# Gibbs-liu/PuzzleNet

Measured on NVIDIA B200. Metric: pairs/sec PuzzleNet fwd B=64 N=1024, higher is better.
Workload: dtype f16x3 (fp16 hi/lo operand planes, 3 tcgen05 MMAs per product, fp32 accumulate)

## Files before the change

puzzlenet_b200/csrc/encoder.cu:

```cuda
#include <stdlib.h>

#include <functional>

#include <cuda_fp16.h>

#include "pz_common.cuh"
#include "se3_math.cuh"

namespace pz {

constexpr int NPTS = 1024;
constexpr int S1 = 512, S2 = 256, KNN = 32;
constexpr int D0 = 64, C1A = 128, C1B = 128, C2A = 256, C2B = 256, LATT = 256, CATT = 256;

struct StemW {
  const float *w1, *b1, *w2, *b2;
  const float *g1, *be1, *m1, *v1, *g2, *be2, *m2, *v2;
};

__global__ void __launch_bounds__(128) stem_kernel(const float* __restrict__ xyz, StemW wa, StemW wb,
                                                   int clouds_per_set, float* __restrict__ out,
                                                   __nv_bfloat16* __restrict__ out_b, __half* __restrict__ out_hi,
                                                   __half* __restrict__ out_lo) {
  __shared__ __align__(16) float w2s[64 * 64];
  __shared__ float w1s[64 * 3], b1s[64], b2s[64];
  const size_t p = (size_t)blockIdx.x * 128 + threadIdx.x;
  const int cloud = (int)(p / NPTS);
  const int n = (int)(p - (size_t)cloud * NPTS);
  const StemW& w = (cloud / clouds_per_set) == 0 ? wa : wb;
  for (int i = threadIdx.x; i < 64 * 64; i += 128) w2s[i] = w.w2[i];
  for (int i = threadIdx.x; i < 64 * 3; i += 128) w1s[i] = w.w1[i];
  if (threadIdx.x < 64) {
    b1s[threadIdx.x] = w.b1[threadIdx.x];
    b2s[threadIdx.x] = w.b2[threadIdx.x];
  }
  __syncthreads();
  const float a1 = w.g1[n] * (1.0f / sqrtf(w.v1[n] + 1e-5f));
  const float c1 = w.be1[n] - w.m1[n] * a1;
  const float a2 = w.g2[n] * (1.0f / sqrtf(w.v2[n] + 1e-5f));
  const float c2 = w.be2[n] - w.m2[n] * a2;
  const float x = xyz[p * 3], y = xyz[p * 3 + 1], z = xyz[p * 3 + 2];
  float h[64];
#pragma unroll
  for (int k = 0; k < 64; ++k) {
    float v = b1s[k];
    v = fmaf(w1s[k * 3 + 0], x, v);
    v = fmaf(w1s[k * 3 + 1], y, v);
    v = fmaf(w1s[k * 3 + 2], z, v);
    h[k] = fmaxf(fmaf(v, a1, c1), 0.f);
  }
  float* o = out + p * 64;
// ... 1206 lines not shown
      prof_mark("attn_out_proj", st);
    }
  }
  {
    float* fg = o.f_global ? o.f_global : s.fglob;
    TcGemm g;
    g.X = cat_b; g.ldx = 1280; g.W[0] = wpa + WP_WOUT; g.W[1] = wpb + WP_WOUT; g.ldw = 1280;
    g.bias[0] = wa.out_b; g.bias[1] = wb.out_b; g.rows_per_wset = B * LATT; g.M = rows; g.Nout = 1024; g.K = 1280;
    if (o.out) {
      g.Yf = o.out; g.ldyf = 1024;
      PZ_TRY(launch_tc_gemm(g, st));
      prof_mark("tail_linear", st);
      rowblock_max_kernel<<<dim3(4, C), 256, 0, st>>>(o.out, 1024, LATT, 1024, C, C, 0, fg, 1024);
      PZ_LAUNCH_CHECK();
      prof_mark("tail_point_max", st);
    } else {
      g.epi = 2; g.Yf = fg; g.ldyf = 1024;
      PZ_TRY(launch_tc_gemm(g, st));
      prof_mark("tail_linear_maxpool", st);
    }
    if (fglob_pair)
      PZ_CUDA(cudaMemcpy2DAsync(fglob_pair, (size_t)E * 1024 * sizeof(float), fg, 1024 * sizeof(float),
                                1024 * sizeof(float), B, cudaMemcpyDeviceToDevice, st));
    if (fglob_pair && E == 2)
      PZ_CUDA(cudaMemcpy2DAsync(fglob_pair + 1024, (size_t)E * 1024 * sizeof(float), fg + (size_t)B * 1024,
                                1024 * sizeof(float), 1024 * sizeof(float), B, cudaMemcpyDeviceToDevice, st));
  }
  return 0;
}


static int encoder_forward_split(const PzEncoderWeights* w, int E, int B, const float* xyz, const int64_t* start1,
                                 const int64_t* start2, const PzEncoderOutputs& o, EncoderScratch& s, float* fglob_pair,
                                 const float** xfeat_out, const AfterStem* after_stem, bool reuse_pack, cudaStream_t st) {
  const int C = E * B;
  const PzEncoderWeights& wa = w[0];
  const PzEncoderWeights& wb = w[E - 1];
  float* xfeat = o.x_feature ? o.x_feature : s.xfeat;
  float* nx2 = o.x2 ? o.x2 : s.nx2;
  if (xfeat_out) *xfeat_out = xfeat;
  typedef __nv_bfloat16 h16;
  h16* xfeat_h[2] = {s.P1, s.P1 + (size_t)C * NPTS * D0};
  float* P1 = s.F1;
  float* P2 = s.F2;
  float* Q1 = s.v;
  float* Q2 = s.r;
  h16* f1f_h[2] = {s.f1f_b, s.Q1};
  h16* cat_h[2] = {s.att_cat_b, reinterpret_cast<h16*>(s.att_cat)};
  h16* qk_h[2] = {s.qk_b, reinterpret_cast<h16*>(s.q)};
  h16* vT_h[2] = {s.vT_b, s.P2};
  h16* r_h[2] = {s.r_b, s.Q2};

  if (!reuse_pack) {
    PackJobs jobs;
    int n = 0;
    auto add = [&](const float* src, int ldi, int rows, int cols, void* dst, int ldo, int mode) {
      if (n < MAX_PACK_JOBS) jobs.j[n] = PackJob{src, dst, ldi, rows, cols, ldo, mode};
      ++n;
    };
    for (int e = 0; e < E; ++e) {
      const PzEncoderWeights& we = w[e];
      for (int pl = 0; pl < 2; ++pl) {
        h16* wp = s.wpack + (size_t)(e * 2 + pl) * WS_TOTAL;
        const int mode = 4 + pl;
        add(we.mlp3_w + 3, 3 + D0, C1A, D0, wp + WS_W3F, D0, mode);
        add(we.mlp4_w, C1A, C1B, C1A, wp + WS_W4, C1A, mode);
        add(we.mlp5_w + 3, 3 + C1B, C2A, C1B, wp + WS_W5F, C1B, mode);
// ... 24 lines not shown
                          {s.wpack + (size_t)(E - 1) * 2 * WS_TOTAL, s.wpack + ((size_t)(E - 1) * 2 + 1) * WS_TOTAL}};
  auto set_w = [&](TcGemm& g, size_t off) {
    g.W[0] = wp_[0][0] + off; g.Wlo[0] = wp_[0][1] + off; g.W[1] = wp_[1][0] + off; g.Wlo[1] = wp_[1][1] + off;
  };

  PZ_CUDA(cudaMemsetAsync(s.tailp, 0, (size_t)3 * C * sizeof(int), st));

  SideStream* ss = nullptr;
  PZ_TRY(side_stream(&ss, st));
  static const bool env_serial = getenv("PZ_SIDE_STREAM") == nullptr || getenv("PZ_NO_SIDE_STREAM") != nullptr;
  const bool serial = env_serial || prof_serial();
  cudaStream_t sg = serial ? st : ss->stream;
  const int gl = serial ? 0 : 1;
  if (!serial) {
    PZ_CUDA(cudaEventRecord(ss->fork, st));
    PZ_CUDA(cudaStreamWaitEvent(sg, ss->fork, 0));
  }
  prof_mark("_side_begin", sg, gl);
  PZ_TRY(launch_fps(xyz, C, NPTS, start1, S1, o.fps1, nullptr, s.nx1, sg));
  prof_mark("fps1", sg, gl);
  PZ_TRY(launch_knn(s.nx1, xyz, C, S1, NPTS, KNN, o.knn1, s.knn1r, nullptr, sg));
  prof_mark("knn1", sg, gl);
  PZ_TRY(launch_centre_proj_f32(s.nx1, wa.mlp3_w, wb.mlp3_w, 3 + D0, B * S1, C * S1, C1A, Q1, sg));
  if (!serial) PZ_CUDA(cudaEventRecord(ss->join_a, sg));
  PZ_TRY(launch_fps(s.nx1, C, S1, start2, S2, o.fps2, nullptr, nx2, sg));
  prof_mark("fps2", sg, gl);
  PZ_TRY(launch_knn(nx2, s.nx1, C, S2, S1, KNN, o.knn2, s.knn2r, nullptr, sg));
  prof_mark("knn2", sg, gl);
  PZ_TRY(launch_centre_proj_f32(nx2, wa.mlp5_w, wb.mlp5_w, 3 + C1B, B * S2, C * S2, C2A, Q2, sg));
  if (!serial) PZ_CUDA(cudaEventRecord(ss->join_b, sg));

  static const bool stem_ffma = getenv("PZ_STEM_FFMA") && getenv("PZ_STEM_FFMA")[0] == '1';
  const int reps = head_reps();
  if (stem_ffma || (C * NPTS) % (128 * reps) != 0) {
    stem_kernel<<<C * NPTS / 128, 128, 0, st>>>(xyz, stem_of(wa), stem_of(wb), B, xfeat, nullptr, nullptr, nullptr);
    PZ_LAUNCH_CHECK();
    PZ_TRY(launch_split_planes(xfeat, D0, (size_t)C * NPTS, D0, xfeat_h[0], xfeat_h[1], D0, st));
  } else {
    PZ_CUDA(cudaFuncSetAttribute(stem_tc_kernel<true>, cudaFuncAttributeMaxDynamicSharedMemorySize, (int)STEM_TC_SMEM));
    PZ_CUDA(launch_pdl(stem_tc_kernel<true>, dim3(C * NPTS / (128 * reps)), dim3(128), STEM_TC_SMEM, st, xyz, stem_of(wa), stem_of(wb),
                       (const __nv_bfloat16*)nullptr, (const __nv_bfloat16*)nullptr, B, reps, xfeat,
                       reinterpret_cast<__nv_bfloat16*>(xfeat_h[0]), reinterpret_cast<__half*>(xfeat_h[1])));
    PZ_LAUNCH_CHECK();
  }
  prof_mark("stem", st);
  {
    TcGemm g;
    g.X = xfeat_h[0]; g.Xlo = xfeat_h[1]; g.ldx = D0; set_w(g, WS_W3F); g.ldw = D0;
    g.bias[0] = wa.mlp3_b; g.bias[1] = wb.mlp3_b; g.rows_per_wset = B * NPTS; g.M = C * NPTS; g.Nout = C1A; g.K = D0;
    g.Yf = P1; g.ldyf = C1A; g.xyz = xyz; g.W1x[0] = wa.mlp3_w; g.W1x[1] = wb.mlp3_w; g.ldw1x = 3 + D0;
    PZ_TRY(launch_split_rowgemm(g, st));
    prof_mark("sg1_layer1", st);
  }
  if (after_stem) PZ_TRY((*after_stem)(xfeat, nullptr));
  if (!serial) PZ_CUDA(cudaStreamWaitEvent(st, ss->join_a, 0));
  prof_mark("_wait_geometry1", st);
  {
    TcGemm g;
    g.Xf = P1; g.ldx = C1A; g.Qf = Q1; g.rows = s.knn1r; set_w(g, WS_W4); g.ldw = C1A;
    g.bias[0] = wa.mlp4_b; g.bias[1] = wb.mlp4_b; g.rows_per_wset = B * S1 * KNN; g.M = C * S1 * KNN; g.Nout = C1B;
    g.K = C1A; g.epi = 1; g.relu = 1; g.Yf = o.f1f; g.ldyf = C1B; g.Yb = f1f_h[0]; g.Yblo = f1f_h[1]; g.ldyb = C1B;
    PZ_TRY(launch_split_gather(g, st));
    prof_mark("sg1_gather_layer2_maxpool", st);
  }
  {
    TcGemm g;
    g.X = f1f_h[0]; g.Xlo = f1f_h[1]; g.ldx = C1B; set_w(g, WS_W5F); g.ldw = C1B;
    g.bias[0] = wa.mlp5_b; g.bias[1] = wb.mlp5_b; g.rows_per_wset = B * S1; g.M = C * S1; g.Nout = C2A; g.K = C1B;
    g.Yf = P2; g.ldyf = C2A; g.xyz = s.nx1; g.W1x[0] = wa.mlp5_w; g.W1x[1] = wb.mlp5_w; g.ldw1x = 3 + C1B;
    PZ_TRY(launch_split_rowgemm(g, st));
    prof_mark("sg2_layer1", st);
  }
  if (!serial) PZ_CUDA(cudaStreamWaitEvent(st, ss->join_b, 0));
  prof_mark("_wait_geometry2", st);
  float* cat_f = o.att_cat;
  {
    TcGemm g;
    g.Xf = P2; g.ldx = C2A; g.Qf = Q2; g.rows = s.knn2r; set_w(g, WS_W6); g.ldw = C2A;
    g.bias[0] = wa.mlp6_b; g.bias[1] = wb.mlp6_b; g.rows_per_wset = B * S2 * KNN; g.M = C * S2 * KNN; g.Nout = C2B;
    g.K = C2A; g.epi = 1; g.relu = 1; g.Yb = cat_h[0] + 4 * CATT; g.Yblo = cat_h[1] + 4 * CATT; g.ldyb = 1280;
    if (cat_f) { g.Yf = cat_f + 4 * CATT; g.ldyf = 1280; }
    else if (o.f2f) { g.Yf = o.f2f; g.ldyf = CATT; }
    PZ_TRY(launch_split_gather(g, st));
    prof_mark("sg2_gather_layer2_maxpool", st);
  }
  if (o.f2f && cat_f)
    PZ_CUDA(cudaMemcpy2DAsync(o.f2f, CATT * sizeof(float), cat_f + 4 * CATT, 1280 * sizeof(float), CATT * sizeof(float),
// ... 51 lines not shown
    g.X = r_h[0]; g.Xlo = r_h[1]; g.ldx = CATT; set_w(g, wl + 384 * CATT); g.ldw = CATT;
    g.bias[0] = wa.o_b[l]; g.bias[1] = wb.o_b[l]; g.rows_per_wset = B * LATT; g.M = rows; g.Nout = CATT; g.K = CATT;
    g.relu = 1; g.Rb = cat_h[0] + xoff; g.Rblo = cat_h[1] + xoff; g.ldrb = 1280;
    g.Yb = cat_h[0] + (size_t)l * CATT; g.Yblo = cat_h[1] + (size_t)l * CATT; g.ldyb = 1280;
    if (cat_f) { g.Yf = cat_f + (size_t)l * CATT; g.ldyf = 1280; }
    PZ_TRY(launch_split_rowgemm(g, st));
    prof_mark("attn_out_proj", st);
  }
  {
    float* fg = o.f_global ? o.f_global : s.fglob;
    TcGemm g;
    g.X = cat_h[0]; g.Xlo = cat_h[1]; g.ldx = 1280; set_w(g, WS_WOUT); g.ldw = 1280;
    g.bias[0] = wa.out_b; g.bias[1] = wb.out_b; g.rows_per_wset = B * LATT; g.M = rows; g.Nout = 1024; g.K = 1280;
    if (o.out) { g.Yf = o.out; g.ldyf = 1024; }
    g.Ymax = s.tailp; g.ldmax = 1024;
    PZ_TRY(launch_split_rowgemm(g, st));
    prof_mark("tail_linear_maxpool", st);
    PZ_CUDA(launch_pdl(rowblock_max_kernel, dim3(4, C), dim3(256), 0, st, (const float*)s.tailp, 1024, LATT / 128, 1024, C, C, 0, fg, 1024));
    PZ_LAUNCH_CHECK();
    prof_mark("tail_point_max", st);
    if (fglob_pair)
      PZ_CUDA(cudaMemcpy2DAsync(fglob_pair, (size_t)E * 1024 * sizeof(float), fg, 1024 * sizeof(float),
                                1024 * sizeof(float), B, cudaMemcpyDeviceToDevice, st));
    if (fglob_pair && E == 2)
      PZ_CUDA(cudaMemcpy2DAsync(fglob_pair + 1024, (size_t)E * 1024 * sizeof(float), fg + (size_t)B * 1024,
                                1024 * sizeof(float), 1024 * sizeof(float), B, cudaMemcpyDeviceToDevice, st));
  }
  return 0;
}

static int encoder_forward_impl(const PzEncoderWeights* w, int E, int B, const float* xyz, const int64_t* start1,
                                const int64_t* start2, int precision, const PzEncoderOutputs& o, void* ws,
                                size_t ws_bytes, float* fglob_pair, const float** xfeat_out, const AfterStem* after_stem,
                                bool reuse_pack, cudaStream_t st) {
  PZ_REQUIRE(E == 1 || E == 2, PZ_ERR_ARG, "encoder: E must be 1 or 2 (got %d)", E);
  PZ_REQUIRE(B >= 1, PZ_ERR_ARG, "encoder: B must be >= 1");
  PZ_REQUIRE(precision == PZ_PREC_FP32 || precision == PZ_PREC_BF16 || precision == PZ_PREC_SPLIT, PZ_ERR_ARG,
             "encoder: unknown precision %d", precision);
  for (int e = 0; e < E; ++e)
    PZ_REQUIRE(encoder_weights_ok(w[e]), PZ_ERR_ARG, "encoder: weight set %d has a null pointer", e);
  const int C = E * B;
  Arena arena(ws, ws_bytes);
  EncoderScratch s;
  encoder_scratch_layout(C, arena, s);
  PZ_REQUIRE(ws && arena.ok(), PZ_ERR_WORKSPACE, "encoder: workspace %zu B < required %zu B", ws_bytes, arena.used);
  if (precision == PZ_PREC_BF16)
    return encoder_forward_bf16(w, E, B, xyz, start1, start2, o, s, fglob_pair, xfeat_out, after_stem, reuse_pack, st);
  if (precision == PZ_PREC_SPLIT)
    return encoder_forward_split(w, E, B, xyz, start1, start2, o, s, fglob_pair, xfeat_out, after_stem, reuse_pack, st);
  const PzEncoderWeights& wa = w[0];
  const PzEncoderWeights& wb = w[E - 1];
  float* xfeat = o.x_feature ? o.x_feature : s.xfeat;
  float* f1f = o.f1f ? o.f1f : s.f1f;
  float* att_cat = o.att_cat ? o.att_cat : s.att_cat;
  float* nx2 = o.x2 ? o.x2 : s.nx2;
  if (xfeat_out) *xfeat_out = xfeat;

  stem_kernel<<<C * NPTS / 128, 128, 0, st>>>(xyz, stem_of(wa), stem_of(wb), B, xfeat, nullptr, nullptr, nullptr);
  PZ_LAUNCH_CHECK();
  prof_mark("stem", st);
  if (after_stem) PZ_TRY((*after_stem)(xfeat, nullptr));

  PZ_TRY(launch_fps(xyz, C, NPTS, start1, S1, o.fps1, nullptr, s.nx1, st));
  prof_mark("fps1", st);
  PZ_TRY(launch_knn(s.nx1, xyz, C, S1, NPTS, KNN, o.knn1, s.knn1r, nullptr, st));
  prof_mark("knn1", st);
  {
    GemmF32 g;
    g.A = xfeat; g.lda = D0; g.W[0] = wa.mlp3_w + 3; g.W[1] = wb.mlp3_w + 3; g.ldw = 3 + D0;
    g.rows_per_wset = B * NPTS; g.Y = s.F1; g.ldy = C1A; g.M = C * NPTS; g.N = C1A; g.K = D0;
    PZ_TRY(launch_gemm_f32(g, st));
    prof_mark("sg1_layer1", st);
  }
  {
    GemmF32 g;
    g.A = s.F1; g.lda = C1A; g.rows = s.knn1r; g.xyz = xyz; g.centers = s.nx1;
    g.W1[0] = wa.mlp3_w; g.W1[1] = wb.mlp3_w; g.b1[0] = wa.mlp3_b; g.b1[1] = wb.mlp3_b; g.ldw1 = 3 + D0;
    g.W[0] = wa.mlp4_w; g.W[1] = wb.mlp4_w; g.bias[0] = wa.mlp4_b; g.bias[1] = wb.mlp4_b; g.ldw = C1A;
    g.rows_per_wset = B * S1 * KNN; g.Y = f1f; g.ldy = C1B; g.M = C * S1 * KNN; g.N = C1B; g.K = C1A;
    g.relu = 1; g.group = 32;
    PZ_TRY(launch_gemm_f32(g, st));
    prof_mark("sg1_gather_layer2_maxpool", st);
// ... 64 lines not shown
      prof_mark("tail_linear_maxpool", st);
      rowblock_max_kernel<<<dim3(4, C), 256, 0, st>>>(s.tailp, 1024, LATT / 128, 1024, C, C, 0, fg, 1024);
    }
    PZ_LAUNCH_CHECK();
    prof_mark("tail_point_max", st);
    if (fglob_pair)
      PZ_CUDA(cudaMemcpy2DAsync(fglob_pair, (size_t)E * 1024 * sizeof(float), fg, 1024 * sizeof(float),
                                1024 * sizeof(float), B, cudaMemcpyDeviceToDevice, st));
    if (fglob_pair && E == 2)
      PZ_CUDA(cudaMemcpy2DAsync(fglob_pair + 1024, (size_t)E * 1024 * sizeof(float), fg + (size_t)B * 1024,
                                1024 * sizeof(float), 1024 * sizeof(float), B, cudaMemcpyDeviceToDevice, st));
  }
  return 0;
}

}

using namespace pz;

extern "C" size_t pz_encoder_workspace_bytes(int E, int B) {
  if (E < 1 || B < 1) return 0;
  Arena a(nullptr, 0);
  EncoderScratch s;
  return align_up(encoder_scratch_layout(E * B, a, s), 256);
}

extern "C" int pz_encoder_forward(const PzEncoderWeights* weights_host, int E, int B, const float* xyz,
                                  const int64_t* start1, const int64_t* start2, int precision,
                                  const PzEncoderOutputs* outputs_host, void* workspace, size_t workspace_bytes,
                                  pz_stream_t stream) {
  PZ_REQUIRE(weights_host && xyz && start1 && start2 && outputs_host, PZ_ERR_ARG, "pz_encoder_forward: null pointer");
  prof_begin(as_stream(stream));
  return encoder_forward_impl(weights_host, E, B, xyz, start1, start2, precision, *outputs_host, workspace,
                              workspace_bytes, nullptr, nullptr, nullptr, false, as_stream(stream));
}

namespace {
struct PredictScratch {
  float *xyz, *fpair, *h0, *h1, *partial, *local, *gmax, *gbias, *tilemax;
  __nv_bfloat16 *ha, *himg, *himg_split;
  int64_t *st1, *st2;
  void* enc;
  size_t enc_bytes, partial_floats;
};
size_t predict_layout(int B, Arena& a, PredictScratch& s) {
  s.xyz = a.take<float>((size_t)2 * B * NPTS * 3);
  s.st1 = a.take<int64_t>((size_t)2 * B);
  s.st2 = a.take<int64_t>((size_t)2 * B);
  s.fpair = a.take<float>((size_t)B * 2048);
  s.h0 = a.take<float>((size_t)B * 1024);
  s.h1 = a.take<float>((size_t)B * 1024);
  s.partial_floats = (size_t)16 * B * 1024;
  s.partial = a.take<float>(s.partial_floats);
  s.local = a.take<float>((size_t)2 * B * NPTS * 64);
  s.gmax = a.take<float>((size_t)B * 64);
  s.gbias = a.take<float>((size_t)2 * B * 64);
  s.tilemax = a.take<float>((size_t)2 * B * 8 * 128);
  s.ha = a.take<__nv_bfloat16>((size_t)2 * B * NPTS * 64);
  s.himg = a.take<__nv_bfloat16>(2 * HEAD_IMG_SET);
  s.himg_split = a.take<__nv_bfloat16>(2 * HEAD_SPLIT_IMG_SET);
  s.enc_bytes = pz_encoder_workspace_bytes(2, B);
  s.enc = a.take<char>(s.enc_bytes);
  return a.used;
}
}

namespace pz {
// ... 98 lines not shown
          jobs.j[n++] = PackJob{pre.w2, wp + 128 * HD_WS, 64, 64, 64, HD_WS, 1};
          jobs.j[n++] = PackJob{seg.w0 + 64, wp + 192 * HD_WS, 128, 64, 64, HD_WS, 1};
          jobs.j[n++] = PackJob{seg.w1, wp + 256 * HD_WS, 64, 32, 64, HD_WS, 1};
          jobs.j[n++] = PackJob{seg.w1, wp + 288 * HD_WS, 64, 32, 64, HD_WS, 3};
        }
        jobs.n = n;
        pack_weights_kernel<<<dim3(16, n), 256, 0, st>>>(jobs);
        PZ_LAUNCH_CHECK();
      }
      head_pre_tc_kernel<<<P / (128 * head_reps()), 128, 0, st>>>(xfeat_b, pre_f, pre_r, s.himg, B, head_reps(), s.ha, s.tilemax);
      PZ_LAUNCH_CHECK();
      head_seg_tc_kernel<<<P / (128 * head_reps()), 128, 0, st>>>(s.ha, seg_f, seg_r, s.himg, B, head_reps(), s.tilemax, de_fpcb,
                                                                  de_mrpcb);
      PZ_LAUNCH_CHECK();
      prof_mark("boundary_heads", st);
      return 0;
    }
    const size_t hl_smem = (3 * 4160 + 64 * 128) * sizeof(float);
    const size_t hs_smem = (64 * 64 + 32 * 64 + 64 + 32 + 64 + 4 + 64 * 128) * sizeof(float);
    PZ_CUDA(cudaFuncSetAttribute(head_seg_kernel, cudaFuncAttributeMaxDynamicSharedMemorySize, (int)hs_smem));
    PZ_CUDA(cudaFuncSetAttribute(head_local_kernel, cudaFuncAttributeMaxDynamicSharedMemorySize, (int)hl_smem));
    head_local_kernel<<<P / 128, 128, hl_smem, st>>>(xfeat, pre_f, pre_r, B, s.local);
    PZ_LAUNCH_CHECK();
    rowblock_max_kernel<<<dim3(1, B), 256, 0, st>>>(s.local + (size_t)B * NPTS * 64, 64, NPTS, 64, B, B, 0, s.gmax, 64);
    PZ_LAUNCH_CHECK();
    seg_bias_kernel<<<dim3(B, 2), 64, 0, st>>>(s.gmax, h.seg_fpc_w[0], h.seg_fpc_b[0], h.seg_rpc_w[0], h.seg_rpc_b[0], B, s.gbias);
    PZ_LAUNCH_CHECK();
    head_seg_kernel<<<P / 128, 128, hs_smem, st>>>(s.local, seg_f, seg_r, s.gbias, B, de_fpcb, de_mrpcb);
    PZ_LAUNCH_CHECK();
    prof_mark("boundary_heads", st);
    return 0;
  };

  const float* xfeat = nullptr;
  PZ_TRY(encoder_forward_impl(enc_host, 2, B, s.xyz, s.st1, s.st2, precision, eo, s.enc, s.enc_bytes, s.fpair,
                              &xfeat, &heads_fn, reuse_pack, st));
  if (need) {
    const size_t ab = (size_t)B * LATT * LATT * sizeof(float), xb = (size_t)B * S2 * 3 * sizeof(float);
    PZ_CUDA(cudaMemcpyAsync(attention_fpc, attn_all, ab, cudaMemcpyDeviceToDevice, st));
    PZ_CUDA(cudaMemcpyAsync(attention_mrpc, attn_all + (size_t)B * LATT * LATT, ab, cudaMemcpyDeviceToDevice, st));
    PZ_CUDA(cudaMemcpyAsync(x2_fpc, x2_all, xb, cudaMemcpyDeviceToDevice, st));
    PZ_CUDA(cudaMemcpyAsync(x2_mrpc, x2_all + (size_t)B * S2 * 3, xb, cudaMemcpyDeviceToDevice, st));
  }
  PZ_TRY(skinny_linear(s.fpair, 2048, h.tf_w[0], h.tf_b[0], B, 1024, 2048, 1, s.h0, 1024, s.partial, s.partial_floats, st));
  PZ_TRY(skinny_linear(s.h0, 1024, h.tf_w[1], h.tf_b[1], B, 512, 1024, 1, s.h1, 512, s.partial, s.partial_floats, st));
  PZ_TRY(skinny_linear(s.h1, 512, h.tf_w[2], h.tf_b[2], B, 512, 512, 1, s.h0, 512, s.partial, s.partial_floats, st));
  PZ_TRY(skinny_linear(s.h0, 512, h.tf_w[3], h.tf_b[3], B, 256, 512, 1, s.h1, 256, s.partial, s.partial_floats, st));
  PZ_TRY(skinny_linear(s.h1, 256, h.tf_w[4], h.tf_b[4], B, 6, 256, 0, out6, 6, s.partial, s.partial_floats, st));
  prof_mark("pose_mlp", st);
  return 0;
}

extern "C" int pz_se3_exp(const float* twist, int B, float* g, pz_stream_t stream) {
  PZ_REQUIRE(twist && g, PZ_ERR_ARG, "pz_se3_exp: null pointer");
  PZ_REQUIRE(B >= 0, PZ_ERR_ARG, "pz_se3_exp: B < 0");
  if (B == 0) return 0;
  se3_exp_kernel<<<(B + 127) / 128, 128, 0, as_stream(stream)>>>(twist, B, g);
  PZ_LAUNCH_CHECK();
  return 0;
}

extern "C" int pz_scaled_dot_attention(const float* q, const float* k, const float* v, int B, int L, int Dk, int Dv,
                                       float* values, float* attention_or_null, pz_stream_t stream) {
  PZ_REQUIRE(q && k && v && values, PZ_ERR_ARG, "pz_scaled_dot_attention: null pointer");
  PZ_REQUIRE(B >= 0, PZ_ERR_ARG, "pz_scaled_dot_attention: B < 0");
  if (B == 0) return 0;
  return launch_attention(q, Dk, k, Dk, v, Dv, B, L, Dk, Dv, nullptr, 0, values, Dv, attention_or_null,
                          attention_or_null ? 1 : 0, as_stream(stream));
}
// ... 230 lines not shown
```

puzzlenet_b200/csrc/heads_split.cu:

```cuda
#include <cuda_fp16.h>

#include "pz_common.cuh"

namespace pz {

namespace {

constexpr int NPTS_H = 1024;
constexpr int HS_WS = 72;
constexpr int PRE_ROWS = 3 * 64, SEG_ROWS = 64 + 32;

__device__ __forceinline__ void mma_f16(float (&d)[4], const uint32_t (&a)[4], uint32_t b0, uint32_t b1) {
  asm volatile("mma.sync.aligned.m16n8k16.row.col.f32.f16.f16.f32 {%0, %1, %2, %3}, {%4, %5, %6, %7}, {%8, %9}, "
               "{%0, %1, %2, %3};"
               : "+f"(d[0]), "+f"(d[1]), "+f"(d[2]), "+f"(d[3])
               : "r"(a[0]), "r"(a[1]), "r"(a[2]), "r"(a[3]), "r"(b0), "r"(b1));
}
__device__ __forceinline__ void split2(float a, float b, uint32_t& hi, uint32_t& lo) {
  uint32_t h;
  asm("cvt.rn.satfinite.f16x2.f32 %0, %1, %2;" : "=r"(h) : "f"(b), "f"(a));
  const float2 hf = __half22float2(*reinterpret_cast<const __half2*>(&h));
  uint32_t l;
  asm("cvt.rn.satfinite.f16x2.f32 %0, %1, %2;" : "=r"(l) : "f"(b - hf.y), "f"(a - hf.x));
  hi = h;
  lo = l;
}
struct Frags {
  uint32_t hi[2][4][4], lo[2][4][4];
};
__device__ __forceinline__ void load_frags(const float* __restrict__ src, int g, int q, Frags& a) {
#pragma unroll
  for (int mt = 0; mt < 2; ++mt)
#pragma unroll
    for (int kt = 0; kt < 4; ++kt) {
      const float* t0 = src + (size_t)(mt * 16 + g) * 64 + kt * 16 + q * 2;
// ... 197 lines not shown
    for (int nt = 0; nt < 4; ++nt) {
      const int col = nt * 8 + q * 2;
      const float bA = b1s[col], bB = b1s[col + 1];
      const float wA0 = w2s[col], wB0 = w2s[col + 1], wA1 = w2s[32 + col], wB1 = w2s[32 + col + 1];
#pragma unroll
      for (int mt = 0; mt < 2; ++mt)
#pragma unroll
        for (int hf = 0; hf < 2; ++hf) {
          const float hA = fmaxf(h1[mt][nt][2 * hf] + bA, 0.f), hB = fmaxf(h1[mt][nt][2 * hf + 1] + bB, 0.f);
          const int j = 2 * mt + hf;
          o[j][0] = fmaf(wA0, hA, fmaf(wB0, hB, o[j][0]));
          o[j][1] = fmaf(wA1, hA, fmaf(wB1, hB, o[j][1]));
        }
    }
#pragma unroll
    for (int j = 0; j < 4; ++j)
#pragma unroll
      for (int c = 0; c < 2; ++c) {
        o[j][c] += __shfl_xor_sync(0xffffffffu, o[j][c], 1);
        o[j][c] += __shfl_xor_sync(0xffffffffu, o[j][c], 2);
      }
    if (q == 0) {
      float* de = set == 0 ? de_a : de_b;
#pragma unroll
      for (int j = 0; j < 4; ++j) {
        const int n = n0 + g + 8 * j;
        de[((size_t)b * 2 + 0) * NPTS_H + n] = o[j][0] + b2s[0];
        de[((size_t)b * 2 + 1) * NPTS_H + n] = o[j][1] + b2s[1];
      }
    }
  }
}

}

int launch_heads_split(const float* xfeat, const HeadMlp3& pre_f, const HeadMlp3& pre_r, const HeadMlp3& seg_f,
                       const HeadMlp3& seg_r, int B, bool reuse_images, void* img, float* local, float* tilemax,
                       float* de_fpcb, float* de_mrpcb, cudaStream_t st) {
  PZ_REQUIRE(xfeat && img && local && tilemax && de_fpcb && de_mrpcb, PZ_ERR_ARG, "heads_split: null pointer");
  __half* im = static_cast<__half*>(img);
  if (!reuse_images) {
    head_images_kernel<<<dim3(8, 2), 256, 0, st>>>(pre_f, pre_r, seg_f, seg_r, im);
    PZ_LAUNCH_CHECK();
  }
  const int P = 2 * B * NPTS_H, reps = 4;
  const size_t pre_smem = (size_t)2 * PRE_ROWS * HS_WS * sizeof(__half) + (3 * 64 + 4 * 64) * sizeof(float);
  PZ_CUDA(cudaFuncSetAttribute(head_pre_split_kernel, cudaFuncAttributeMaxDynamicSharedMemorySize, (int)pre_smem));
  PZ_CUDA(launch_pdl(head_pre_split_kernel, dim3(P / (128 * reps)), dim3(128), pre_smem, st, xfeat, pre_f, pre_r, (const __half*)im, B, reps,
                     local, tilemax));
  PZ_LAUNCH_CHECK();
  PZ_CUDA(launch_pdl(head_seg_split_kernel, dim3(P / (128 * reps)), dim3(128), 0, st, (const float*)local, seg_f, seg_r, (const __half*)im, B,
                     reps, (const float*)tilemax, de_fpcb, de_mrpcb));
  PZ_LAUNCH_CHECK();
  return 0;
}

}
```

puzzlenet_b200/csrc/pz_common.cuh:

```cuda
#pragma once
#include <cuda_bf16.h>
#include <cuda_runtime.h>
#include <stdint.h>
#include <stdio.h>
#include <stdarg.h>
#include <utility>

#include "../../include/puzzlenet_b200.h"

namespace pz {

char* error_buffer();
int fail(int code, const char* fmt, ...);

#define PZ_REQUIRE(cond, code, ...)                      \
  do {                                                   \
    if (!(cond)) return ::pz::fail((code), __VA_ARGS__); \
  } while (0)

#define PZ_CUDA(expr)                                                                   \
  do {                                                                                  \
    cudaError_t _e = (expr);                                                            \
    if (_e != cudaSuccess)                                                              \
      return ::pz::fail((int)_e, "%s failed: %s (%s:%d)", #expr, cudaGetErrorString(_e), \
// ... 143 lines not shown
  const float* Qf = nullptr;
};
int launch_tc_gemm(const TcGemm& g, cudaStream_t st);
int launch_split_rowgemm(const TcGemm& g, cudaStream_t st);
int launch_split_gather(const TcGemm& g, cudaStream_t st);
int launch_split_planes(const float* in, size_t ldi, size_t rows, int cols, void* hi, void* lo, size_t ldo, cudaStream_t st);
struct AttnSplit {
  const void *qk_hi = nullptr, *qk_lo = nullptr, *vT_hi = nullptr, *vT_lo = nullptr, *x_hi = nullptr, *x_lo = nullptr;
  int ldx = 0;
  void *r_hi = nullptr, *r_lo = nullptr;
  float* attn = nullptr;
  int attn_mode = 0;
  const void *wo_hi[2] = {nullptr, nullptr}, *wo_lo[2] = {nullptr, nullptr};
  const float* bo[2] = {nullptr, nullptr};
  int clouds_per_set = 0;
  void *y_hi = nullptr, *y_lo = nullptr;
  int ldy = 0;
  float* yf = nullptr;
  int ldyf = 0;
  const void *wqkv_hi[2] = {nullptr, nullptr}, *wqkv_lo[2] = {nullptr, nullptr};
  const float* bqkv[2] = {nullptr, nullptr};
  void *qk2_hi = nullptr, *qk2_lo = nullptr, *vT2_hi = nullptr, *vT2_lo = nullptr;
  const int* dep_flags = nullptr;
  int* sig_flags = nullptr;
};
int launch_attention_split(const AttnSplit& p, int clouds, cudaStream_t st);
struct HeadMlp3 {
  const float *w0, *b0, *w1, *b1, *w2, *b2;
};
constexpr size_t HEAD_SPLIT_IMG_SET = (size_t)(2 * 3 * 64 + 2 * (64 + 32)) * 72;
int launch_heads_split(const float* xfeat, const HeadMlp3& pre_f, const HeadMlp3& pre_r, const HeadMlp3& seg_f,
                       const HeadMlp3& seg_r, int B, bool reuse_images, void* img, float* local, float* tilemax,
                       float* de_fpcb, float* de_mrpcb, cudaStream_t st);
int launch_tc_rowgemm(const TcGemm& g, cudaStream_t st);
int launch_attention_tc(const __nv_bfloat16* qk, const __nv_bfloat16* vT, const __nv_bfloat16* x, int ldx, int clouds,
                        __nv_bfloat16* r, float* attn, int attn_mode, cudaStream_t st);
struct AttnLayerTc {
  int nlayers = 1;
  const __nv_bfloat16* x = nullptr;
  int ldx = 0;
  const __nv_bfloat16* wimg[2] = {nullptr, nullptr};
  const float* bqkv[2] = {nullptr, nullptr};
  const float* bo[2][4] = {{nullptr, nullptr, nullptr, nullptr}, {nullptr, nullptr, nullptr, nullptr}};
  int clouds_per_set = 0;
  __nv_bfloat16* yb = nullptr;
  int ldyb = 0;
  size_t yb_layer_stride = 0;
  float* yf = nullptr;
  int ldyf = 0;
  size_t yf_layer_stride = 0;
  float* attn = nullptr;
  int attn_mode[4] = {0, 0, 0, 0};
  long long* prof = nullptr;
};
int launch_attention_layer_tc(const AttnLayerTc& p, int clouds, cudaStream_t st);
constexpr size_t ATTN_WIMG_ELEMS = 20 * 128 * 64;
int launch_attn_weight_image(const float* src, int rows, int row_off, __nv_bfloat16* img, cudaStream_t st);
int launch_cvt_bf16(const float* in, int ldi, int rows, int cols, __nv_bfloat16* out, int ldo, cudaStream_t st);

}
```

Baseline: 46250.

## Fuse stem MLP and head pre-MLP into one persistent tcgen05 front kernel

Adds a persistent front kernel that, per 128-point tile, runs the two stem layers and the three head pre-MLP layers through tcgen05 split-fp16 MMAs, keeping the intermediate feature in shared memory. It writes the xfeat hi/lo planes, local features and per-tile max directly, replacing the separate stem kernel and head_pre kernel and their global round-trip of xfeat. The head seg kernel now launches right after the first row GEMM. This trades extra register and shared-memory pressure and a serial per-tile MMA chain for fewer launches and less memory traffic. The old path stays available through an environment variable.

```diff
diff --git a/puzzlenet_b200/csrc/encoder.cu b/puzzlenet_b200/csrc/encoder.cu
--- a/puzzlenet_b200/csrc/encoder.cu
+++ b/puzzlenet_b200/csrc/encoder.cu
@@ -12,11 +12,6 @@
 constexpr int NPTS = 1024;
 constexpr int S1 = 512, S2 = 256, KNN = 32;
 constexpr int D0 = 64, C1A = 128, C1B = 128, C2A = 256, C2B = 256, LATT = 256, CATT = 256;
-
-struct StemW {
-  const float *w1, *b1, *w2, *b2;
-  const float *g1, *be1, *m1, *v1, *g2, *be2, *m2, *v2;
-};
 
 __global__ void __launch_bounds__(128) stem_kernel(const float* __restrict__ xyz, StemW wa, StemW wb,
                                                    int clouds_per_set, float* __restrict__ out,
@@ -1289,7 +1284,8 @@
 
 static int encoder_forward_split(const PzEncoderWeights* w, int E, int B, const float* xyz, const int64_t* start1,
                                  const int64_t* start2, const PzEncoderOutputs& o, EncoderScratch& s, float* fglob_pair,
-                                 const float** xfeat_out, const AfterStem* after_stem, bool reuse_pack, cudaStream_t st) {
+                                 const float** xfeat_out, const AfterStem* after_stem, const FrontSplit* front,
+                                 bool reuse_pack, cudaStream_t st) {
   const int C = E * B;
   const PzEncoderWeights& wa = w[0];
   const PzEncoderWeights& wb = w[E - 1];
@@ -1380,7 +1376,11 @@
 
   static const bool stem_ffma = getenv("PZ_STEM_FFMA") && getenv("PZ_STEM_FFMA")[0] == '1';
   const int reps = head_reps();
-  if (stem_ffma || (C * NPTS) % (128 * reps) != 0) {
+  if (front) {
+    PZ_REQUIRE(E == 2, PZ_ERR_ARG, "encoder: the split front needs both weight sets");
+    PZ_TRY(launch_front_split(xyz, stem_of(wa), stem_of(wb), *front, B, o.x_feature, xfeat_h[0], xfeat_h[1], st));
+    prof_mark("front", st);
+  } else if (stem_ffma || (C * NPTS) % (128 * reps) != 0) {
     stem_kernel<<<C * NPTS / 128, 128, 0, st>>>(xyz, stem_of(wa), stem_of(wb), B, xfeat, nullptr, nullptr, nullptr);
     PZ_LAUNCH_CHECK();
     PZ_TRY(launch_split_planes(xfeat, D0, (size_t)C * NPTS, D0, xfeat_h[0], xfeat_h[1], D0, st));
@@ -1391,7 +1391,7 @@
                        reinterpret_cast<__nv_bfloat16*>(xfeat_h[0]), reinterpret_cast<__half*>(xfeat_h[1])));
     PZ_LAUNCH_CHECK();
   }
-  prof_mark("stem", st);
+  if (!front) prof_mark("stem", st);
   {
     TcGemm g;
     g.X = xfeat_h[0]; g.Xlo = xfeat_h[1]; g.ldx = D0; set_w(g, WS_W3F); g.ldw = D0;
@@ -1400,7 +1400,12 @@
     PZ_TRY(launch_split_rowgemm(g, st));
     prof_mark("sg1_layer1", st);
   }
-  if (after_stem) PZ_TRY((*after_stem)(xfeat, nullptr));
+  if (front) {
+    PZ_TRY(launch_front_seg_split(*front, B, st));
+    prof_mark("head_seg", st);
+  } else if (after_stem) {
+    PZ_TRY((*after_stem)(xfeat, nullptr));
+  }
   if (!serial) PZ_CUDA(cudaStreamWaitEvent(st, ss->join_a, 0));
   prof_mark("_wait_geometry1", st);
   {
@@ -1518,7 +1523,7 @@
 static int encoder_forward_impl(const PzEncoderWeights* w, int E, int B, const float* xyz, const int64_t* start1,
                                 const int64_t* start2, int precision, const PzEncoderOutputs& o, void* ws,
                                 size_t ws_bytes, float* fglob_pair, const float** xfeat_out, const AfterStem* after_stem,
-                                bool reuse_pack, cudaStream_t st) {
+                                const FrontSplit* front, bool reuse_pack, cudaStream_t st) {
   PZ_REQUIRE(E == 1 || E == 2, PZ_ERR_ARG, "encoder: E must be 1 or 2 (got %d)", E);
   PZ_REQUIRE(B >= 1, PZ_ERR_ARG, "encoder: B must be >= 1");
   PZ_REQUIRE(precision == PZ_PREC_FP32 || precision == PZ_PREC_BF16 || precision == PZ_PREC_SPLIT, PZ_ERR_ARG,
@@ -1533,7 +1538,8 @@
   if (precision == PZ_PREC_BF16)
     return encoder_forward_bf16(w, E, B, xyz, start1, start2, o, s, fglob_pair, xfeat_out, after_stem, reuse_pack, st);
   if (precision == PZ_PREC_SPLIT)
-    return encoder_forward_split(w, E, B, xyz, start1, start2, o, s, fglob_pair, xfeat_out, after_stem, reuse_pack, st);
+    return encoder_forward_split(w, E, B, xyz, start1, start2, o, s, fglob_pair, xfeat_out, after_stem, front, reuse_pack,
+                                 st);
   const PzEncoderWeights& wa = w[0];
   const PzEncoderWeights& wb = w[E - 1];
   float* xfeat = o.x_feature ? o.x_feature : s.xfeat;
@@ -1664,7 +1670,7 @@
   PZ_REQUIRE(weights_host && xyz && start1 && start2 && outputs_host, PZ_ERR_ARG, "pz_encoder_forward: null pointer");
   prof_begin(as_stream(stream));
   return encoder_forward_impl(weights_host, E, B, xyz, start1, start2, precision, *outputs_host, workspace,
-                              workspace_bytes, nullptr, nullptr, nullptr, false, as_stream(stream));
+                              workspace_bytes, nullptr, nullptr, nullptr, nullptr, false, as_stream(stream));
 }
 
 namespace {
@@ -1829,9 +1835,12 @@
     return 0;
   };
 
+  static const bool front_legacy = getenv("PZ_FRONT_LEGACY") && getenv("PZ_FRONT_LEGACY")[0] == '1';
+  const FrontSplit front = {pre_f, pre_r, seg_f, seg_r, s.himg_split, s.local, s.tilemax, de_fpcb, de_mrpcb, reuse_pack};
+  const bool use_front = precision == PZ_PREC_SPLIT && !front_legacy;
   const float* xfeat = nullptr;
   PZ_TRY(encoder_forward_impl(enc_host, 2, B, s.xyz, s.st1, s.st2, precision, eo, s.enc, s.enc_bytes, s.fpair,
-                              &xfeat, &heads_fn, reuse_pack, st));
+                              &xfeat, use_front ? nullptr : &heads_fn, use_front ? &front : nullptr, reuse_pack, st));
   if (need) {
     const size_t ab = (size_t)B * LATT * LATT * sizeof(float), xb = (size_t)B * S2 * 3 * sizeof(float);
     PZ_CUDA(cudaMemcpyAsync(attention_fpc, attn_all, ab, cudaMemcpyDeviceToDevice, st));
diff --git a/puzzlenet_b200/csrc/heads_split.cu b/puzzlenet_b200/csrc/heads_split.cu
--- a/puzzlenet_b200/csrc/heads_split.cu
+++ b/puzzlenet_b200/csrc/heads_split.cu
@@ -1,6 +1,9 @@
 #include <cuda_fp16.h>
 
+#include <algorithm>
+
 #include "pz_common.cuh"
+#include "tc_common.cuh"
 
 namespace pz {
 
@@ -264,6 +267,241 @@
   }
 }
 
+constexpr int FR_THREADS = 128;
+constexpr uint32_t FR_A = 128 * 128;
+constexpr uint32_t FR_W = 64 * 128;
+constexpr uint32_t FR_W_OFF = 2 * FR_A;
+constexpr uint32_t FR_SMALL_OFF = FR_W_OFF + 8 * FR_W;
+constexpr size_t FR_SMEM = 1024 + FR_SMALL_OFF + 64 * sizeof(float4) + (64 + 3 * 64 + 2 * 64) * sizeof(float) + 16;
+constexpr uint32_t FR_IDESC = (1u << 4) | ((uint32_t)(64 >> 3) << 17) | ((uint32_t)(128 >> 4) << 24);
+
+template <bool Sat>
+__device__ __forceinline__ void put_row(uint8_t* a_hi, int r, const float (&v)[64]) {
+#pragma unroll
+  for (int c = 0; c < 8; ++c) {
+    uint32_t h[4], l[4];
+#pragma unroll
+    for (int e = 0; e < 4; ++e) {
+      const float x0 = v[c * 8 + 2 * e], x1 = v[c * 8 + 2 * e + 1];
+      if (Sat) {
+        split2(x0, x1, h[e], l[e]);
+      } else {
+        const __half2 hh = __floats2half2_rn(x0, x1);
+        const float2 hf = __half22float2(hh);
+        const __half2 hl = __floats2half2_rn(x0 - hf.x, x1 - hf.y);
+        h[e] = *reinterpret_cast<const uint32_t*>(&hh);
+        l[e] = *reinterpret_cast<const uint32_t*>(&hl);
+      }
+    }
+    const uint32_t off = tc::sw128(r, c);
+    *reinterpret_cast<uint4*>(a_hi + off) = make_uint4(h[0], h[1], h[2], h[3]);
+    *reinterpret_cast<uint4*>(a_hi + FR_A + off) = make_uint4(l[0], l[1], l[2], l[3]);
+  }
+}
+
+__global__ void __launch_bounds__(FR_THREADS, 2) front_split_kernel(const float* __restrict__ xyz, StemW sa, StemW sb, HeadMlp3 pa,
+                                                                    HeadMlp3 pb, const __half* __restrict__ img, int B,
+                                                                    float* __restrict__ xfeat, __half* __restrict__ xf_hi,
+                                                                    __half* __restrict__ xf_lo, float* __restrict__ local,
+                                                                    float* __restrict__ tilemax) {
+  using namespace tc;
+  extern __shared__ __align__(1024) uint8_t fr_smem_raw[];
+  const uint32_t base = (smem_u32(fr_smem_raw) + 1023u) & ~1023u;
+  uint8_t* sm = fr_smem_raw + (base - smem_u32(fr_smem_raw));
+  float4* w1p = reinterpret_cast<float4*>(sm + FR_SMALL_OFF);
+  float* b2s = reinterpret_cast<float*>(w1p + 64);
+  float* pbs = b2s + 64;
+  float* cmax = pbs + 3 * 64;
+  const uint32_t bar = smem_u32(cmax + 2 * 64), tmem_slot = bar + 8;
+  const int tid = threadIdx.x, warp = tid >> 5;
+  const int ctas_per_set = gridDim.x / 2, set = (int)blockIdx.x / ctas_per_set, rank = (int)blockIdx.x - set * ctas_per_set;
+  const int tiles_per_set = B * (NPTS_H / 128);
+  const StemW& sw = set == 0 ? sa : sb;
+  const HeadMlp3& pw = set == 0 ? pa : pb;
+
+  if (tid == 0) {
+    mbar_init(bar, 1);
+    asm volatile("fence.mbarrier_init.release.cluster;" ::: "memory");
+  }
+  if (warp == 0) {
+    asm volatile("tcgen05.alloc.cta_group::1.sync.aligned.shared::cta.b32 [%0], %1;" ::"r"(tmem_slot), "r"(64) : "memory");
+    asm volatile("tcgen05.relinquish_alloc_permit.cta_group::1.sync.aligned;" ::: "memory");
+  }
+  pdl_enter();
+  {
+    const __half* src = img + (size_t)set * HEAD_SPLIT_IMG_SET;
+#pragma unroll
+    for (int j = 0; j < 2 * 3 * 64 * 8 / FR_THREADS; ++j) {
+      const int i = j * FR_THREADS + tid, c = i & 7, n = (i >> 3) & 63, l = (i >> 9) % 3, p = i / (3 * 512);
+      cp_async16(base + FR_W_OFF + (uint32_t)(2 * (l + 1) + p) * FR_W + sw128(n, c),
+                 src + (size_t)(p * PRE_ROWS + l * 64 + n) * HS_WS + c * 8);
+    }
+    cp_async_commit();
+  }
+  {
+    float f[4][8];
+#pragma unroll
+    for (int j = 0; j < 4; ++j)
+#pragma unroll
+      for (int e = 0; e < 8; ++e) f[j][e] = sw.w2[(j * FR_THREADS + tid) * 8 + e];
+#pragma unroll
+    for (int j = 0; j < 4; ++j) {
+      const int i = j * FR_THREADS + tid, n = i >> 3, c = i & 7;
+      uint32_t h[4], l[4];
+#pragma unroll
+      for (int e = 0; e < 4; ++e) {
+        const __half2 hh = __floats2half2_rn(f[j][2 * e], f[j][2 * e + 1]);
+        const float2 hf = __half22float2(hh);
+        const __half2 hl = __floats2half2_rn(f[j][2 * e] - hf.x, f[j][2 * e + 1] - hf.y);
+        h[e] = *reinterpret_cast<const uint32_t*>(&hh);
+        l[e] = *reinterpret_cast<const uint32_t*>(&hl);
+      }
+      *reinterpret_cast<uint4*>(sm + FR_W_OFF + sw128(n, c)) = make_uint4(h[0], h[1], h[2], h[3]);
+      *reinterpret_cast<uint4*>(sm + FR_W_OFF + FR_W + sw128(n, c)) = make_uint4(l[0], l[1], l[2], l[3]);
+    }
+  }
+  if (tid < 64) {
+    w1p[tid] = make_float4(sw.w1[tid * 3], sw.w1[tid * 3 + 1], sw.w1[tid * 3 + 2], sw.b1[tid]);
+    b2s[tid] = sw.b2[tid];
+    pbs[tid] = pw.b0[tid];
+    pbs[64 + tid] = pw.b1[tid];
+    pbs[128 + tid] = pw.b2[tid];
+  }
+  cp_async_wait<0>();
+  fence_proxy_async();
+  tc_fence_before();
+  __syncthreads();
+  tc_fence_after();
+  const uint32_t tmem = *reinterpret_cast<volatile uint32_t*>(sm + (tmem_slot - base));
+  const uint32_t trow = tmem + ((uint32_t)(warp * 32) << 16);
+  uint8_t* a_s = sm;
+  uint32_t phase = 0;
+
+  auto mma_layer = [&](int l) {
+    fence_proxy_async();
+    tc_fence_before();
+    __syncthreads();
+    if (warp == 0) {
+      tc_fence_after();
+      if (elect_one()) {
+        const uint64_t a_hi = make_desc(base), a_lo = make_desc(base + FR_A);
+        const uint64_t b_hi = make_desc(base + FR_W_OFF + 2 * l * FR_W), b_lo = make_desc(base + FR_W_OFF + (2 * l + 1) * FR_W);
+#pragma unroll
+        for (int k4 = 0; k4 < 4; ++k4) {
+          umma_bf16(tmem, a_hi + 2 * k4, b_hi + 2 * k4, FR_IDESC, k4 != 0);
+          umma_bf16(tmem, a_hi + 2 * k4, b_lo + 2 * k4, FR_IDESC, 1);
+          umma_bf16(tmem, a_lo + 2 * k4, b_hi + 2 * k4, FR_IDESC, 1);
+        }
+        umma_commit(bar);
+      }
+      __syncwarp();
+    }
+  };
+  auto wait_acc = [&](float (&v)[64]) {
+    mbar_wait(bar, phase);
+    phase ^= 1;
+    tc_fence_after();
+    tmem_ld64(trow, v);
+    tc_fence_before();
+  };
+
+  float in[11];
+  auto load_inputs = [&](int t) {
+    const int tile = set * tiles_per_set + t, n = (tile & 7) * 128 + tid;
+    const size_t p = (size_t)tile * 128 + tid;
+    in[0] = xyz[p * 3]; in[1] = xyz[p * 3 + 1]; in[2] = xyz[p * 3 + 2];
+    in[3] = sw.g1[n]; in[4] = sw.v1[n]; in[5] = sw.be1[n]; in[6] = sw.m1[n];
+    in[7] = sw.g2[n]; in[8] = sw.v2[n]; in[9] = sw.be2[n]; in[10] = sw.m2[n];
+  };
+  if (rank < tiles_per_set) load_inputs(rank);
+
+#pragma unroll 1
+  for (int t = rank; t < tiles_per_set; t += ctas_per_set) {
+    const int tile = set * tiles_per_set + t;
+    const size_t p0 = (size_t)tile * 128, p = p0 + tid;
+    float v[64];
+    const float x = in[0], y = in[1], z = in[2];
+    const float a1 = in[3] * (1.0f / sqrtf(in[4] + 1e-5f)), c1 = in[5] - in[6] * a1;
+    const float a2 = in[7] * (1.0f / sqrtf(in[8] + 1e-5f)), c2 = in[9] - in[10] * a2;
+    if (t + ctas_per_set < tiles_per_set) load_inputs(t + ctas_per_set);
+#pragma unroll
+    for (int k = 0; k < 64; ++k) {
+      const float4 w = w1p[k];
+      float s = w.w;
+      s = fmaf(w.x, x, s); s = fmaf(w.y, y, s); s = fmaf(w.z, z, s);
+      v[k] = fmaxf(fmaf(s, a1, c1), 0.f);
+    }
+    put_row<false>(a_s, tid, v);
+    mma_layer(0);
+    wait_acc(v);
+#pragma unroll
+    for (int k = 0; k < 64; ++k) v[k] = fmaxf(fmaf(v[k] + b2s[k], a2, c2), 0.f);
+    if (xfeat) {
+      float4* o = reinterpret_cast<float4*>(xfeat + p * 64);
+#pragma unroll
+      for (int c = 0; c < 16; ++c) o[c] = make_float4(v[4 * c], v[4 * c + 1], v[4 * c + 2], v[4 * c + 3]);
+    }
+    put_row<false>(a_s, tid, v);
+    mma_layer(1);
+#pragma unroll
+    for (int it = 0; it < 8; ++it) {
+      const int idx = it * FR_THREADS + tid, r = idx >> 3, c = idx & 7;
+      *reinterpret_cast<uint4*>(xf_hi + (p0 + r) * 64 + c * 8) = *reinterpret_cast<const uint4*>(a_s + sw128(r, c));
+      *reinterpret_cast<uint4*>(xf_lo + (p0 + r) * 64 + c * 8) = *reinterpret_cast<const uint4*>(a_s + FR_A + sw128(r, c));
+    }
+    __syncthreads();
+#pragma unroll 1
+    for (int l = 0; l < 2; ++l) {
+      wait_acc(v);
+#pragma unroll
+      for (int k = 0; k < 64; ++k) v[k] = fmaxf(v[k] + pbs[l * 64 + k], 0.f);
+      put_row<true>(a_s, tid, v);
+      mma_layer(l + 2);
+    }
+    wait_acc(v);
+#pragma unroll
+    for (int c = 0; c < 16; ++c)
+      *reinterpret_cast<float4*>(a_s + tid * 256 + ((c ^ (tid & 15)) << 4)) =
+          make_float4(v[4 * c] + pbs[128 + 4 * c], v[4 * c + 1] + pbs[128 + 4 * c + 1], v[4 * c + 2] + pbs[128 + 4 * c + 2],
+                      v[4 * c + 3] + pbs[128 + 4 * c + 3]);
+    __syncthreads();
+#pragma unroll
+    for (int it = 0; it < 16; ++it) {
+      const int idx = it * FR_THREADS + tid, r = idx >> 4, c = idx & 15;
+      *reinterpret_cast<float4*>(local + (p0 + r) * 64 + c * 4) = *reinterpret_cast<const float4*>(a_s + r * 256 + ((c ^ (r & 15)) << 4));
+    }
+    {
+      const int col = tid & 63, h = tid >> 6;
+      float m = -INFINITY;
+#pragma unroll 8
+      for (int r = h * 64; r < h * 64 + 64; ++r)
+        m = fmaxf(m, *reinterpret_cast<const float*>(a_s + r * 256 + (((col >> 2) ^ (r & 15)) << 4) + (col & 3) * 4));
+      cmax[h * 64 + col] = m;
+    }
+    __syncthreads();
+    if (tid < 64) tilemax[(size_t)tile * 64 + tid] = fmaxf(cmax[tid], cmax[64 + tid]);
+  }
+  tc_fence_before();
+  __syncthreads();
+  if (warp == 0) asm volatile("tcgen05.dealloc.cta_group::1.sync.aligned.b32 %0, %1;" ::"r"(tmem), "r"(64) : "memory");
+}
+
+}
+
+static int launch_head_images(const HeadMlp3& pre_f, const HeadMlp3& pre_r, const HeadMlp3& seg_f, const HeadMlp3& seg_r,
+                              __half* img, cudaStream_t st) {
+  head_images_kernel<<<dim3(8, 2), 256, 0, st>>>(pre_f, pre_r, seg_f, seg_r, img);
+  PZ_LAUNCH_CHECK();
+  return 0;
+}
+
+static int launch_head_seg(const float* local, const HeadMlp3& seg_f, const HeadMlp3& seg_r, const __half* img, int B,
+                           const float* tilemax, float* de_fpcb, float* de_mrpcb, cudaStream_t st) {
+  const int P = 2 * B * NPTS_H, reps = 4;
+  PZ_CUDA(launch_pdl(head_seg_split_kernel, dim3(P / (128 * reps)), dim3(128), 0, st, local, seg_f, seg_r, img, B, reps,
+                     tilemax, de_fpcb, de_mrpcb));
+  PZ_LAUNCH_CHECK();
+  return 0;
 }
 
 int launch_heads_split(const float* xfeat, const HeadMlp3& pre_f, const HeadMlp3& pre_r, const HeadMlp3& seg_f,
@@ -271,20 +509,32 @@
                        float* de_fpcb, float* de_mrpcb, cudaStream_t st) {
   PZ_REQUIRE(xfeat && img && local && tilemax && de_fpcb && de_mrpcb, PZ_ERR_ARG, "heads_split: null pointer");
   __half* im = static_cast<__half*>(img);
-  if (!reuse_images) {
-    head_images_kernel<<<dim3(8, 2), 256, 0, st>>>(pre_f, pre_r, seg_f, seg_r, im);
-    PZ_LAUNCH_CHECK();
-  }
+  if (!reuse_images) PZ_TRY(launch_head_images(pre_f, pre_r, seg_f, seg_r, im, st));
   const int P = 2 * B * NPTS_H, reps = 4;
   const size_t pre_smem = (size_t)2 * PRE_ROWS * HS_WS * sizeof(__half) + (3 * 64 + 4 * 64) * sizeof(float);
   PZ_CUDA(cudaFuncSetAttribute(head_pre_split_kernel, cudaFuncAttributeMaxDynamicSharedMemorySize, (int)pre_smem));
   PZ_CUDA(launch_pdl(head_pre_split_kernel, dim3(P / (128 * reps)), dim3(128), pre_smem, st, xfeat, pre_f, pre_r, (const __half*)im, B, reps,
                      local, tilemax));
   PZ_LAUNCH_CHECK();
-  PZ_CUDA(launch_pdl(head_seg_split_kernel, dim3(P / (128 * reps)), dim3(128), 0, st, (const float*)local, seg_f, seg_r, (const __half*)im, B,
-                     reps, (const float*)tilemax, de_fpcb, de_mrpcb));
+  return launch_head_seg(local, seg_f, seg_r, im, B, tilemax, de_fpcb, de_mrpcb, st);
+}
+
+int launch_front_split(const float* xyz, const StemW& stem_f, const StemW& stem_r, const FrontSplit& f, int B, float* xfeat,
+                       void* xf_hi, void* xf_lo, cudaStream_t st) {
+  PZ_REQUIRE(xyz && xf_hi && xf_lo && f.img && f.local && f.tilemax, PZ_ERR_ARG, "front_split: null pointer");
+  __half* im = static_cast<__half*>(f.img);
+  if (!f.reuse_images) PZ_TRY(launch_head_images(f.pre_f, f.pre_r, f.seg_f, f.seg_r, im, st));
+  PZ_CUDA(cudaFuncSetAttribute(front_split_kernel, cudaFuncAttributeMaxDynamicSharedMemorySize, (int)FR_SMEM));
+  const int ctas_per_set = std::min(B * (NPTS_H / 128), kNumSMs);
+  PZ_CUDA(launch_pdl(front_split_kernel, dim3(2 * ctas_per_set), dim3(FR_THREADS), FR_SMEM, st, xyz, stem_f, stem_r, f.pre_f, f.pre_r,
+                     (const __half*)im, B, xfeat, static_cast<__half*>(xf_hi), static_cast<__half*>(xf_lo), f.local, f.tilemax));
   PZ_LAUNCH_CHECK();
   return 0;
 }
 
-}
+int launch_front_seg_split(const FrontSplit& f, int B, cudaStream_t st) {
+  PZ_REQUIRE(f.de_fpcb && f.de_mrpcb, PZ_ERR_ARG, "front_split: null pointer");
+  return launch_head_seg(f.local, f.seg_f, f.seg_r, static_cast<const __half*>(f.img), B, f.tilemax, f.de_fpcb, f.de_mrpcb, st);
+}
+
+}
diff --git a/puzzlenet_b200/csrc/pz_common.cuh b/puzzlenet_b200/csrc/pz_common.cuh
--- a/puzzlenet_b200/csrc/pz_common.cuh
+++ b/puzzlenet_b200/csrc/pz_common.cuh
@@ -199,6 +199,19 @@
 int launch_heads_split(const float* xfeat, const HeadMlp3& pre_f, const HeadMlp3& pre_r, const HeadMlp3& seg_f,
                        const HeadMlp3& seg_r, int B, bool reuse_images, void* img, float* local, float* tilemax,
                        float* de_fpcb, float* de_mrpcb, cudaStream_t st);
+struct StemW {
+  const float *w1, *b1, *w2, *b2;
+  const float *g1, *be1, *m1, *v1, *g2, *be2, *m2, *v2;
+};
+struct FrontSplit {
+  HeadMlp3 pre_f, pre_r, seg_f, seg_r;
+  void* img;
+  float *local, *tilemax, *de_fpcb, *de_mrpcb;
+  bool reuse_images;
+};
+int launch_front_split(const float* xyz, const StemW& stem_f, const StemW& stem_r, const FrontSplit& f, int B, float* xfeat,
+                       void* xf_hi, void* xf_lo, cudaStream_t st);
+int launch_front_seg_split(const FrontSplit& f, int B, cudaStream_t st);
 int launch_tc_rowgemm(const TcGemm& g, cudaStream_t st);
 int launch_attention_tc(const __nv_bfloat16* qk, const __nv_bfloat16* vT, const __nv_bfloat16* x, int ldx, int clouds,
                         __nv_bfloat16* r, float* attn, int attn_mode, cudaStream_t st);
```

Measured after the change: 47320, median of 6. +2.3%, better.
